# MKimiSH/video-filler

Hardware: AMD Instinct MI355X
Metric: netG+netD fwd+bwd images/sec, 128x128 center-mask (higher is better)
Workload: dtype f32

## Files before the change

video-filler_amd/csrc/vf_pgemm.hip:

```cpp
#include <algorithm>
#include <cstdlib>

#include "vf_device.h"

template <int NPL>
__global__ __launch_bounds__(256) void k_planes_split(const float* __restrict__ x, __bf16* __restrict__ planes, int64_t n4,
                                                      int64_t pstride) {
  for (int64_t i = blockIdx.x * (int64_t)blockDim.x + threadIdx.x; i < n4; i += (int64_t)gridDim.x * blockDim.x) {
    if constexpr (NPL == 1) {
      *(u32x2*)(planes + 4 * i) = vf_round4(((const f32x4*)x)[i]);
    } else {
      u32x2 o[3];
      vf_split3(((const f32x4*)x)[i], o);
#pragma unroll
      for (int q = 0; q < 3; ++q) *(u32x2*)(planes + q * pstride + 4 * i) = o[q];
    }
  }
}
__global__ __launch_bounds__(256) void k_weight_planes(const float* __restrict__ w, __bf16* __restrict__ nat, __bf16* __restrict__ tr,
                                                       int d0, int d1, int64_t pstride, int npl) {
  __shared__ float tile[32][33];
  const int t0 = blockIdx.x * 32, tap = blockIdx.y, u0 = blockIdx.z * 32;
  const int tx = threadIdx.x & 31, ty = threadIdx.x >> 5;
  for (int j = ty; j < 32; j += 8) {
// ... 511 lines not shown
    for (int g = 0; g < CH / 16; ++g) {
      const int cs = g & 1;
      if (g + 1 < CH / 16) read_frag(g + 1, cs ^ 1);
      __builtin_amdgcn_sched_barrier(0);
      if constexpr (NPL == 3) {
        acc[0][0] = __builtin_amdgcn_mfma_f32_32x32x16_bf16(a[cs][1], b[cs][1], acc[0][0], 0, 0, 0);
        acc[0][0] = __builtin_amdgcn_mfma_f32_32x32x16_bf16(a[cs][0], b[cs][2], acc[0][0], 0, 0, 0);
        acc[0][0] = __builtin_amdgcn_mfma_f32_32x32x16_bf16(a[cs][2], b[cs][0], acc[0][0], 0, 0, 0);
        acc[0][0] = __builtin_amdgcn_mfma_f32_32x32x16_bf16(a[cs][0], b[cs][1], acc[0][0], 0, 0, 0);
        acc[0][0] = __builtin_amdgcn_mfma_f32_32x32x16_bf16(a[cs][1], b[cs][0], acc[0][0], 0, 0, 0);
      }
      acc[0][0] = __builtin_amdgcn_mfma_f32_32x32x16_bf16(a[cs][0], b[cs][0], acc[0][0], 0, 0, 0);
      __builtin_amdgcn_sched_barrier(0);
    }
  };

  float pre_d[16], pre_x[16];
  const bool fin_tile = p.ksplit == 1;
  const bool want_d = fin_tile && p.dmask != nullptr, want_x = fin_tile && p.st.mode == 2;
#pragma unroll
  for (int r = 0; r < 16; ++r) {
    pre_d[r] = 1.f;
    pre_x[r] = 0.f;
  }
  if (want_d || want_x) {
    const int n = n0 + wn + lr;
    const int bw = 2 * (n >> 6) + (n & 1), bb = (n >> 1) & 31, wpp = p.N >> 5;
#pragma unroll
    for (int r = 0; r < 16; ++r) {
      const int m = m0 + wm + (r & 3) + 8 * (r >> 2) + 4 * lh;
      const int mx = m & (Mw - 1), my = (m >> p.lgMw) & (Mh - 1), b = m >> (p.lgMw + p.lgMh);
      const int64_t pix = ((int64_t)b * p.outH + (my * p.osy + ooy0)) * p.outW + (mx * p.osx + oox0);
      if (want_d) pre_d[r] = p.dbits ? (float)((p.dbits[pix * wpp + bw] >> bb) & 1u) : p.dmask[pix * p.N + n];
      if (want_x) pre_x[r] = p.st.x[pix * p.N + n];
    }
  }

  dma_step(ch0, VfIntC<0>{}, 0, ch0 < ch1);
  static_assert(NTAPS % 2 == 0, "the two LDS stages alternate with the tap parity");
  for (int ch = ch0; ch < ch1; ++ch) {
    const bool more = ch + 1 < ch1;
    asm volatile("" : "+s"(rowA), "+s"(colA), "+s"(w0), "+s"(rowW), "+s"(colW));
    vf_static_for<NTAPS>([&](auto T) {
      constexpr int t = decltype(T)::value;
      constexpr int buf = NBUF == 2 ? (t & 1) : 0, nbuf = NBUF == 2 ? (buf ^ 1) : 0;
      auto next_stage = [&]() {
        if (!(p.dbg & 1)) {
          if constexpr (t + 1 < NTAPS)
            dma_step(ch, VfIntC<t + 1>{}, nbuf, true);
          else
            dma_step(ch + 1, VfIntC<0>{}, nbuf, more);
        }
      };
      asm volatile("s_waitcnt vmcnt(0)\n\ts_barrier" ::: "memory");
      __builtin_amdgcn_sched_barrier(0);
      if constexpr (NBUF == 2) next_stage();
      __builtin_amdgcn_sched_barrier(0);
      if (!(p.dbg & 4)) compute_step(buf);
      if constexpr (NBUF == 1) {
        asm volatile("s_barrier" ::: "memory");
        next_stage();
      }
    });
  }
  asm volatile("s_waitcnt vmcnt(0)\n\ts_barrier" ::: "memory");
  pg_epilogue<1, 1, WAVES_M, BN, true>(p, acc, (float*)smem, m0, n0, wm, wn, lane, tid, wave / WAVES_N, bx, ks, ooy0, oox0, ph, pw, true,
                                       pre_d, pre_x);
}

template <int CPB>
__global__ __launch_bounds__(512) void k_pconv_patch_tr(const PGemm p) {
  constexpr int PR = CPB == 4 ? 10 : 9, PW = 18, NSLOT = PR * PW, NG = (NSLOT + 7) / 8;
  constexpr int AGW = (NG + 7) / 8;
  constexpr int PATCH_PL = NG * 8 * 128, PATCH_BYTES = 3 * PATCH_PL;
  constexpr int W_PL = 64 * 128, WBUF = 3 * W_PL;
  constexpr int NS = 4 * CPB;
  __shared__ __attribute__((aligned(1024))) unsigned char smem[PATCH_BYTES + 2 * WBUF + 2 * 4 * 64 * 4];
  float* red = (float*)(smem + PATCH_BYTES + 2 * WBUF);

  const int tid = threadIdx.x, lane = tid & 63;
  const int wave = __builtin_amdgcn_readfirstlane(tid >> 6);
  const int wm = (wave >> 1) * 32, wn = (wave & 1) * 32;
  const int lr = lane & 31, lh = lane >> 5;
  int lid = vf_xcd_remap(blockIdx.x, gridDim.x);
  const int n0 = 64 * (lid % p.gn);
  lid /= p.gn;
  int ph_blk = 0;
  if constexpr (CPB == 2) {
    ph_blk = lid & 1;
    lid >>= 1;
  }
  const int tiles_x = p.Wi >> 4, tiles_y = p.Hi >> 3;
  const int tx = lid % tiles_x, ty = (lid / tiles_x) % tiles_y, b = lid / (tiles_x * tiles_y);
  const int ry0 = 8 * ty, rx0 = 16 * tx;
  const int bx = lid;
  auto patch_sw = [](int px) { return (px >> 1) & 7; };

  unsigned a_byte[AGW], a_lds[AGW];
#pragma unroll
  for (int i = 0; i < AGW; ++i) {
    const int grp = wave + 8 * i;
    const int sl = 8 * grp + (lane >> 3);
    const int py = sl / PW, px = sl - py * PW;
    const int il = ry0 - 1 + (CPB == 2 ? ph_blk : 0) + py, jl = rx0 - 1 + px;
    const bool ok = grp < NG && sl < NSLOT && (unsigned)il < (unsigned)p.Hi && (unsigned)jl < (unsigned)p.Wi;
    const int oct = (lane & 7) ^ patch_sw(px);
    a_byte[i] = ok ? 2u * (unsigned)(((b * p.Hi + il) * p.Wi + jl) * p.C + 8 * oct) : VF_OOB;
    a_lds[i] = (unsigned)(grp * 8 * 128);
  }
  const int wrow = 8 * wave + (lane >> 3);
  const unsigned w_byte = 2u * (unsigned)((n0 + wrow) * 16 * p.C + 8 * ((lane & 7) ^ ((wrow >> 1) & 7)));
  const unsigned w_lds = (unsigned)(wave * 8 * 128);
  const __amdgpu_buffer_rsrc_t rsA = vf_rsrc(p.A, p.a_bytes), rsW = vf_rsrc(p.W, p.w_bytes);
  const unsigned lds0 = (unsigned)(uintptr_t)(__attribute__((address_space(3))) void*)smem;
  unsigned szero;
  asm volatile("s_mov_b32 %0, 0" : "=s"(szero));

  auto dma_patch = [&](int ch) {
    const unsigned cb = 128u * (unsigned)ch;
#pragma unroll
    for (int i = 0; i < AGW; ++i) {
      if (wave + 8 * i < NG) {
#pragma unroll
        for (int q = 0; q < 3; ++q)
          pg_dma16(lds0 + (unsigned)(q * PATCH_PL) + a_lds[i], a_byte[i] == VF_OOB ? VF_OOB : a_byte[i] + cb, rsA, szero + q * p.a_ps);
      }
    }
  };
  auto dma_w = [&](int ch, auto STEP, int buf) {
    constexpr int s_ = decltype(STEP)::value, cls = s_ >> 2, th = (s_ >> 1) & 1, tw = s_ & 1;
    const int ph = CPB == 4 ? (cls >> 1) : ph_blk, pw = CPB == 4 ? (cls & 1) : cls;
    const int kh = 3 - ph - 2 * th, kw = 3 - pw - 2 * tw;
    const unsigned tW = 2u * (unsigned)((kh * 4 + kw) * p.C) + 128u * (unsigned)ch;
#pragma unroll
    for (int q = 0; q < 3; ++q)
      pg_dma16(lds0 + (unsigned)(PATCH_BYTES + buf * WBUF + q * W_PL) + w_lds, w_byte, rsW, q * p.w_ps + tW);
  };

  f32x16 acc[CPB];
#pragma unroll
  for (int c = 0; c < CPB; ++c)
#pragma unroll
    for (int r = 0; r < 16; ++r) acc[c][r] = 0.f;

  const int arow = wm + lr;
  const int apy = arow >> 4, apx = arow & 15;
  int slot00 = apy * PW + apx;
  const int brow = wn + lr;
  unsigned b_off0 = (unsigned)(brow * 128);
  const unsigned b_sw = (unsigned)((brow >> 1) & 7);
  auto compute_step = [&](auto STEP, int buf) {
    constexpr int s_ = decltype(STEP)::value, cls = s_ >> 2, th = (s_ >> 1) & 1, tw = s_ & 1;
    const int ph = CPB == 4 ? (cls >> 1) : 0, pw = CPB == 4 ? (cls & 1) : cls;
    const int slot = slot00 + (ph + th) * PW + pw + tw;
    const unsigned a_off0 = (unsigned)(slot * 128), a_sw = (unsigned)patch_sw(apx + pw + tw);
    const unsigned char* wb = smem + PATCH_BYTES + buf * WBUF;
    bf16x8 a[2][3], bb[2][3];
    auto read_frag = [&](int g, int set) {
      const unsigned o = (unsigned)(2 * g + lh);
#pragma unroll
      for (int q = 0; q < 3; ++q) {
        a[set][q] = *(const bf16x8*)(smem + q * PATCH_PL + a_off0 + ((o ^ a_sw) << 4));
        bb[set][q] = *(const bf16x8*)(wb + q * W_PL + b_off0 + ((o ^ b_sw) << 4));
      }
    };
    read_frag(0, 0);
#pragma unroll
    for (int g = 0; g < 4; ++g) {
      const int cs = g & 1;
      if (g + 1 < 4) read_frag(g + 1, cs ^ 1);
      __builtin_amdgcn_sched_barrier(0);
      acc[cls] = __builtin_amdgcn_mfma_f32_32x32x16_bf16(a[cs][1], bb[cs][1], acc[cls], 0, 0, 0);
      acc[cls] = __builtin_amdgcn_mfma_f32_32x32x16_bf16(a[cs][0], bb[cs][2], acc[cls], 0, 0, 0);
      acc[cls] = __builtin_amdgcn_mfma_f32_32x32x16_bf16(a[cs][2], bb[cs][0], acc[cls], 0, 0, 0);
      acc[cls] = __builtin_amdgcn_mfma_f32_32x32x16_bf16(a[cs][0], bb[cs][1], acc[cls], 0, 0, 0);
      acc[cls] = __builtin_amdgcn_mfma_f32_32x32x16_bf16(a[cs][1], bb[cs][0], acc[cls], 0, 0, 0);
      acc[cls] = __builtin_amdgcn_mfma_f32_32x32x16_bf16(a[cs][0], bb[cs][0], acc[cls], 0, 0, 0);
      __builtin_amdgcn_sched_barrier(0);
    }
  };

  const int n = wn + lr;
  const int N = p.N;
  const int stm = p.st.mode;
  const bool want_d = p.dmask != nullptr, want_x = stm == 2;
  const float bv = p.bias ? p.bias[n0 + n] : 0.f;
  const float sv = stm ? p.st.vec[(stm == 2 ? (bx / p.st.tiles_per_group) * N : 0) + n0 + n] : 0.f;
  const float neg = p.act == VF_ACT_LRELU ? p.slope : (p.act == VF_ACT_RELU ? 0.f : 1.f);
  const float dneg = p.dact == VF_ACT_LRELU ? p.dslope : (p.dact == VF_ACT_RELU ? 0.f : 1.f);
  const unsigned ybytes = (unsigned)(p.out_elems * 4);
  const __amdgpu_buffer_rsrc_t rsY = vf_rsrc(p.Y, ybytes), rsD = vf_rsrc(p.dbits ? (const void*)p.dbits : (const void*)p.dmask, p.dbits ? ybytes / 32 : ybytes),
                               rsX = vf_rsrc(p.st.x, ybytes);
  unsigned pix0 = (unsigned)(((b * p.outH + 2 * (ry0 + 2 * (wave >> 1))) * p.outW) + 2 * (rx0 + 4 * lh));
  const unsigned ostride = (unsigned)(2 * p.outW);
  float pre_d[16], pre_x[16];
  auto pixel = [&](int r, int ph, int pw) -> unsigned {
    return pix0 + (unsigned)(ph * p.outW + pw) + (unsigned)(r >> 3) * ostride + (unsigned)(2 * ((r & 3) + 8 * ((r >> 2) & 1)));
  };
  auto elem = [&](int r, int ph, int pw) -> unsigned { return pixel(r, ph, pw) * (unsigned)N + (unsigned)(n0 + n); };
  auto prefetch_epi = [&](int ph, int pw) {
#pragma unroll
    for (int r = 0; r < 16; ++r) {
      const unsigned px_ = pixel(r, ph, pw), e = px_ * (unsigned)N + (unsigned)(n0 + n);
      pre_d[r] = 1.f;
      pre_x[r] = 0.f;
      if (want_d) {
        if (p.dbits)
          pre_d[r] = (float)((__builtin_amdgcn_raw_buffer_load_b32(rsD, 4u * (px_ * (unsigned)(N >> 5) + (unsigned)(2 * (n0 >> 6) + (n & 1))), 0, 0) >> ((n >> 1) & 31)) & 1u);
        else pre_d[r] = __builtin_bit_cast(float, __builtin_amdgcn_raw_buffer_load_b32(rsD, 4u * e, 0, 0));
      }
      if (want_x) pre_x[r] = __builtin_bit_cast(float, __builtin_amdgcn_raw_buffer_load_b32(rsX, 4u * e, 0, 0));
    }
  };
  auto epilogue = [&](auto CLS, int ph, int pw) {
    constexpr int cls = decltype(CLS)::value;
    float st1[1] = {0.f}, st2[1] = {0.f};
#pragma unroll
    for (int r = 0; r < 16; ++r) {
      float v = acc[cls][r] + bv;
      v = v * (v > 0.f ? 1.f : neg);
      if (want_d) v = v * (pre_d[r] > 0.f ? 1.f : dneg);
      if (stm == 1) {
        const float d = v - sv;
        st1[0] += d;
        st2[0] += d * d;
      } else if (stm == 2) {
        st1[0] += v;
        st2[0] += v * (pre_x[r] - sv);
      }
      acc[cls][r] = v;
    }
    if (stm) vf_bn_tile_partials<1, 4, 64>(p.st, st1, st2, red, wave >> 1, wn, lane, tid, n0, N, bx, (ph << 1) | pw);
  };
  auto store_class = [&](auto CLS, int ph, int pw) {
    constexpr int cls = decltype(CLS)::value;
#pragma unroll
    for (int r = 0; r < 16; ++r) {
      const float v = acc[cls][r];
      if (!(p.dbg & 8)) __builtin_amdgcn_raw_buffer_store_b32(__builtin_bit_cast(unsigned, v), rsY, 4u * elem(r, ph, pw), 0, 0);
    }
  };

  const int nch = p.nchunks;
  dma_patch(0);
  dma_w(0, VfIntC<0>{}, 0);
  for (int ch = 0; ch < nch; ++ch) {
    const bool last = ch + 1 == nch;
    asm volatile("" : "+v"(slot00), "+v"(b_off0), "+v"(pix0));
    vf_static_for<NS>([&](auto S) {
      constexpr int s_ = decltype(S)::value, buf = s_ & 1, cls = s_ >> 2, tap = s_ & 3;
      const int ph = CPB == 4 ? (cls >> 1) : ph_blk, pw = CPB == 4 ? (cls & 1) : cls;
      asm volatile("s_waitcnt vmcnt(0)\n\ts_barrier" ::: "memory");
      __builtin_amdgcn_sched_barrier(0);
      if (!(p.dbg & 1)) {
        if constexpr (s_ + 1 < NS) dma_w(ch, VfIntC<s_ + 1>{}, buf ^ 1);
        else if (!last) dma_w(ch + 1, VfIntC<0>{}, buf ^ 1);
      }
      if (last && tap == 0 && (want_d || want_x)) prefetch_epi(ph, pw);
      __builtin_amdgcn_sched_barrier(0);
      if (!(p.dbg & 4)) compute_step(S, buf);
      if (last && tap == 3) epilogue(VfIntC<cls>{}, ph, pw);
    });
    if (!last) {
      asm volatile("s_barrier" ::: "memory");
      dma_patch(ch + 1);
    }
  }
  vf_static_for<CPB>([&](auto C) {
    constexpr int cls = decltype(C)::value;
    store_class(C, CPB == 4 ? (cls >> 1) : ph_blk, CPB == 4 ? (cls & 1) : cls);
  });
}

template <int MODE, bool TR = false>
__global__ __launch_bounds__(512) void k_pconv_patch_g(const PGemm p) {
  static_assert(!TR || MODE != 0, "the transposed form serves whole-map tiles (8 x 16 regions of larger maps: k_pconv_patch_tr)");
  constexpr int NS = TR ? 4 : 16;
  constexpr int PW = 17;
  constexpr int NSLOT = MODE == 0 ? 9 * PW : 130;
  constexpr int NG = (NSLOT + 7) / 8, AGW = (NG + 7) / 8;
  constexpr int PL = NG * 8 * 128;
  constexpr int W_PL = 64 * 128, WBUF = 3 * W_PL;
  constexpr int OFF_LO = 4 * PL, OFF_W = 5 * PL;
  __shared__ __attribute__((aligned(1024))) unsigned char smem[5 * PL + 2 * WBUF];
  float* red = (float*)(smem + OFF_W);

  const int tid = threadIdx.x, lane = tid & 63;
  const int wave = __builtin_amdgcn_readfirstlane(tid >> 6);
  const int wm = (wave >> 1) * 32, wn = (wave & 1) * 32;
  const int lr = lane & 31, lh = lane >> 5;
  const int ntiles = p.gm * p.gn * p.gz;
  int lid = vf_xcd_remap(blockIdx.x, ntiles);
  int ph = 0, pw = 0;
  if constexpr (TR) {
    ph = (lid >> 1) & 1;
    pw = lid & 1;
    lid >>= 2;
  }
  const int bx = lid % p.gm, byz = lid / p.gm;
  const int n0 = (byz % p.gn) * 64;
  const int ks = byz / p.gn;
  const int cps = p.nchunks / p.ksplit;
  const int ch0 = ks * cps;
  const int Wo = 1 << p.lgMw, Ho = 1 << p.lgMh;

  int b_img = 0, oy0 = 0, ox0 = 0;
  if constexpr (MODE == 0) {
    const int tiles_x = Wo >> 4, tiles_y = Ho >> 3;
    const int tx = bx % tiles_x, ty = (bx / tiles_x) % tiles_y;
    b_img = bx / (tiles_x * tiles_y);
    oy0 = 8 * ty;
    ox0 = 16 * tx;
  }
  constexpr int HW = MODE == 1 ? 64 : 16, LW = MODE == 1 ? 3 : 2;

  unsigned a_byte[AGW], a_ok[AGW], a_lds[AGW];
#pragma unroll
  for (int i = 0; i < AGW; ++i) {
    const int grp = wave + 8 * i;
    const int sl = 8 * grp + (lane >> 3);
    a_lds[i] = (unsigned)(grp * 8 * 128);
    if constexpr (MODE == 0) {
      const int r = sl / PW, c = sl - r * PW;
      const int y00 = 2 * (oy0 + r) - 1, x00 = 2 * (ox0 + c) - 1;
      const int oct = (lane & 7) ^ (c & 7);
      a_byte[i] = 2u * (unsigned)(((b_img * p.Hi + y00) * p.Wi + x00) * p.C + 8 * oct);
      unsigned ok = 0;
#pragma unroll
      for (int cls = 0; cls < 4; ++cls)
        if ((unsigned)(y00 + (cls >> 1)) < (unsigned)p.Hi && (unsigned)(x00 + (cls & 1)) < (unsigned)p.Wi) ok |= 1u << cls;
      a_ok[i] = (grp < NG && sl < NSLOT) ? ok : 0u;
    } else {
      const int g = sl >> (2 * LW), ii = (sl >> LW) & (Wo - 1), jj = sl & (Wo - 1);
      const int oct = (lane & 7) ^ ((sl >> 1) & 7);
      const int img = bx * (128 / HW) + g;
      if constexpr (TR) a_byte[i] = 2u * (unsigned)(((img * p.Hi + ii) * p.Wi + jj) * p.C + 8 * oct);
      else a_byte[i] = 2u * (unsigned)(((img * p.Hi + 2 * ii + 1) * p.Wi + 2 * jj + 1) * p.C + 8 * oct);
      a_ok[i] = (grp < NG && sl < 128) ? 15u : 0u;
    }
  }
  const int wrow = 8 * wave + (lane >> 3);
  const unsigned w_byte = 2u * (unsigned)((n0 + wrow) * 16 * p.C + 8 * ((lane & 7) ^ ((wrow >> 1) & 7)));
  const unsigned w_lds = (unsigned)(wave * 8 * 128);
  const __amdgpu_buffer_rsrc_t rsA = vf_rsrc(p.A, p.a_bytes), rsW = vf_rsrc(p.W, p.w_bytes);
  const unsigned lds0 = (unsigned)(uintptr_t)(__attribute__((address_space(3))) void*)smem;
  unsigned szero;
  asm volatile("s_mov_b32 %0, 0" : "=s"(szero));
  int rowA = 2 * p.Wi * p.C, colA = 2 * p.C;

  auto dma_patch_plane = [&](int ch, int cls, int pb, auto Q, bool live) {
    constexpr int q = decltype(Q)::value;
    const int cth = cls >> 1, ctw = cls & 1;
    const unsigned cb = 128u * (unsigned)ch + (TR ? 0u : (unsigned)(MODE == 0 ? cth * rowA + ctw * colA : -(cth * rowA + ctw * colA)));
    const unsigned dst = lds0 + (unsigned)(q == 2 ? OFF_LO : (2 * pb + q) * PL);
// ... 373 lines not shown
          acc[nt] = __builtin_amdgcn_mfma_f32_32x32x16_bf16(a1[0], b1[0][nt], acc[nt], 0, 0, 0);
        }
      }
    } else {
    bf16x8 a[2][NPL], b[2][NPL][2];
    auto read_frag = [&](int g, int set) {
#pragma unroll
      for (int q = 0; q < NPL; ++q) {
        a[set][q] = pg_tr_frag(base + q * PL_SZ, wm, 16 * g, lane);
#pragma unroll
        for (int nt = 0; nt < 2; ++nt) b[set][q][nt] = pg_tr_frag(base + q * PL_SZ + TILE, wn + 32 * nt, 16 * g, lane);
      }
    };
    read_frag(0, 0);
#pragma unroll
    for (int g = 0; g < BK / 16; ++g) {
      const int cs = g & 1;
      if (g + 1 < BK / 16) read_frag(g + 1, cs ^ 1);
      __builtin_amdgcn_sched_barrier(0);
#pragma unroll
      for (int nt = 0; nt < 2; ++nt) {
        if constexpr (NPL == 3) {
          acc[nt] = __builtin_amdgcn_mfma_f32_32x32x16_bf16(a[cs][1], b[cs][1][nt], acc[nt], 0, 0, 0);
          acc[nt] = __builtin_amdgcn_mfma_f32_32x32x16_bf16(a[cs][0], b[cs][2][nt], acc[nt], 0, 0, 0);
          acc[nt] = __builtin_amdgcn_mfma_f32_32x32x16_bf16(a[cs][2], b[cs][0][nt], acc[nt], 0, 0, 0);
          acc[nt] = __builtin_amdgcn_mfma_f32_32x32x16_bf16(a[cs][0], b[cs][1][nt], acc[nt], 0, 0, 0);
          acc[nt] = __builtin_amdgcn_mfma_f32_32x32x16_bf16(a[cs][1], b[cs][0][nt], acc[nt], 0, 0, 0);
        }
        acc[nt] = __builtin_amdgcn_mfma_f32_32x32x16_bf16(a[cs][0], b[cs][0][nt], acc[nt], 0, 0, 0);
      }
      __builtin_amdgcn_sched_barrier(0);
    }
    }
  };

  if (fed32) {
    for (int kt = kt0; kt < kt1; ++kt) {
      stage_fp32(kt);
      __syncthreads();
      compute_stage();
      __syncthreads();
    }
  } else {
    for (int kt = kt0; kt < kt1; ++kt) {
      dma_stage(kt);
      asm volatile("s_waitcnt vmcnt(0)\n\ts_barrier" ::: "memory");
      __builtin_amdgcn_sched_barrier(0);
      compute_stage();
      asm volatile("s_barrier" ::: "memory");
    }
  }

  const int lr = lane & 31, lh = lane >> 5;
  const int64_t total = (int64_t)p.Nu * Ncols;
  float* out = p.out + (p.ksplit > 1 ? (int64_t)ks * total : 0);
  const bool acc_old = p.ksplit == 1 && p.beta != 0.f;
#pragma unroll
  for (int r = 0; r < 16; ++r) {
    const int n = n0 + wm + (r & 3) + 8 * (r >> 2) + 4 * lh;
    if (n >= p.Nu) continue;
#pragma unroll
    for (int nt = 0; nt < 2; ++nt) {
      const int64_t idx = (int64_t)n * Ncols + j0 + wn + nt * 32 + lr;
      float v = acc[nt][r];
      if (acc_old) v += p.beta * out[idx];
      out[idx] = v;
    }
  }
}

int vf_internal_pwgrad_group(vf_ctx* ctx, const VfPWGradGroup& G, int blocks, const char* name, double flops) {
  if (ctx->mfma_bf16 == 1)
    VF_LAUNCH_TIMED(ctx, "pwgrad_group_128x128x32_bf16", flops, 0.0, (k_pwgrad_group<1, 2>), dim3((unsigned)blocks), dim3(512), G);
  else
    VF_LAUNCH_TIMED(ctx, name, flops, 0.0, (k_pwgrad_group<3, 1>), dim3((unsigned)blocks), dim3(512), G);
  VF_LAUNCH_CHECK();
  return 0;
}

static int g_gather_patch = 1;
static int g_scatter_patch = 1;
VF_API int vf_pconv_set_routing(int gather_patch, int scatter_patch) {
  if (gather_patch >= 0) g_gather_patch = gather_patch != 0;
  if (scatter_patch >= 0) g_scatter_patch = scatter_patch != 0;
  return 0;
}

typedef void (*PgKernel)(PGemm);

template <int BM, int NTAPS>
static PgKernel pg_dma_kernel(bool one_plane, bool one_stage) {
  if (one_plane) return k_pconv_dma<BM, 64, NTAPS, 2, 1>;
  return one_stage ? k_pconv_dma<BM, 64, NTAPS, 1> : k_pconv_dma<BM, 64, NTAPS, 2>;
}

template <int BM, int WM, int NTAPS>
static PgKernel pg_reg_kernel(int ch) {
  return ch == 64 ? k_pconv<BM, 64, WM, 32, NTAPS, 64> : k_pconv<BM, 64, WM, 32, NTAPS, 32>;
}

static int launch_pconv(vf_ctx* ctx, PGemm& g, int ntaps, VfConvExtras* ex) {
  const int zpar = g.parity ? 4 : 1;
  const int ch = g.C % 64 == 0 ? 64 : 32;
  g.nchunks = g.C / ch;
  constexpr int bn = 64;
  const bool dma_shape = ch == 64 && g.N % bn == 0;
  const int bm = dma_shape ? (g.M % 128 == 0 ? 128 : 64) : (vf_cdiv(g.M, 128) * vf_cdiv(g.N, bn) * zpar >= 1024 ? 128 : 64);
  const bool use_dma = dma_shape && g.M % bm == 0;
  const int gm = (int)vf_cdiv(g.M, bm), gn = (int)vf_cdiv(g.N, bn);
  const int64_t blocks = (int64_t)gm * gn * zpar;
  constexpr int SPLIT_BLOCKS = 340;
  int ksplit = 1;
  if (blocks < SPLIT_BLOCKS * 3 / 4 && g.nchunks >= 2) {
    ksplit = (int)std::min<int64_t>(g.nchunks, vf_cdiv(SPLIT_BLOCKS, blocks));
    const size_t slab_bytes = (size_t)g.out_elems * sizeof(float);
    while (ksplit > 1 && (size_t)ksplit * slab_bytes > vf_ws_avail(ctx)) --ksplit;
    while (ksplit > 1 && g.nchunks % ksplit != 0) --ksplit;
  }
  g.ksplit = ksplit;
  g.slab = ksplit > 1 ? (float*)vf_ws_ptr(ctx) : nullptr;
  g.gm = gm; g.gn = gn; g.gz = zpar * ksplit;
  const unsigned nt = (unsigned)(blocks * ksplit);
  const bool slab_st = vf_plan_bn_stats(ex, g, bm, gm, zpar);
  const bool one_plane = ctx->mfma_bf16 == 1;
  VF_REQUIRE(!one_plane || use_dma, "vf_pconv: in the bf16-operand mode the planes path serves whole 64-channel / 64-row tiles only "
             "(vf_pconv_supported_in_mode)");

  const char* taps = ntaps == 16 ? "t16" : "t4";
  const double fl = 2.0 * (double)g.M * g.N * (double)ntaps * g.C * zpar;
  const double dby = (double)g.a_bytes + (double)g.w_bytes + 4.0 * (double)g.out_elems * ksplit +
                     (g.dmask ? (g.dbits ? 0.125 : 4.0) * (double)g.out_elems : 0.0) + (g.st.mode == 2 ? 4.0 * (double)g.out_elems : 0.0);
  char name[64];
  PgKernel kern;
  dim3 grid(nt), block(bm == 128 ? 512 : 256);
  double by = dby;
  const int Ho = 1 << g.lgMh, Wo = 1 << g.lgMw;
  const int gmode = (Wo % 16 == 0 && Ho % 8 == 0) ? 0 : (Ho == 8 && Wo == 8) ? 1 : (Ho == 4 && Wo == 4) ? 2 : -1;
  if (use_dma && one_plane) {
    snprintf(name, sizeof(name), "pconv_dma_%dx%dx64_%s_bf16", bm, bn, taps);
    kern = bm == 128 ? (ntaps == 16 ? pg_dma_kernel<128, 16>(true, false) : pg_dma_kernel<128, 4>(true, false))
                     : (ntaps == 16 ? pg_dma_kernel<64, 16>(true, false) : pg_dma_kernel<64, 4>(true, false));
  } else if (use_dma && g_scatter_patch && ntaps == 4 && g.parity && ksplit == 1 && bm == 128 && g.Wi % 16 == 0 && g.Hi % 8 == 0 &&
             (g.act == VF_ACT_NONE || g.act == VF_ACT_LRELU || g.act == VF_ACT_RELU) &&
             g.out_elems * 4 < ((int64_t)1 << 31)) {
    const unsigned tiles = (unsigned)(g.M / 128), slices = (unsigned)(g.N / 64);
    const int cpb = tiles * slices >= 512 ? 4 : 2;
    snprintf(name, sizeof(name), "pconv_patch_128x64_t4_c%d", cpb);
    grid = dim3(tiles * slices * (cpb == 2 ? 2u : 1u));
    kern = cpb == 4 ? k_pconv_patch_tr<4> : k_pconv_patch_tr<2>;
  } else if (use_dma && g_gather_patch && ntaps == 16 && !g.parity && bm == 128 && g.sy == 2 && g.sx == 2 && gmode >= 0) {
    snprintf(name, sizeof(name), "pconv_patchg_128x64_t16_m%d", gmode);
    kern = gmode == 0 ? k_pconv_patch_g<0> : gmode == 1 ? k_pconv_patch_g<1> : k_pconv_patch_g<2>;
  } else if (use_dma && g_scatter_patch && ntaps == 4 && g.parity && bm == 128 && nt < 512 &&
             ((g.Hi == 8 && g.Wi == 8) || (g.Hi == 4 && g.Wi == 4))) {
    const int mode = g.Hi == 8 ? 1 : 2;
    snprintf(name, sizeof(name), "pconv_patchg_128x64_t4_m%d", mode);
    kern = mode == 1 ? k_pconv_patch_g<1, true> : k_pconv_patch_g<2, true>;
  } else if (use_dma) {
    const bool one_stage = bm == 128 && nt >= 512;
    snprintf(name, sizeof(name), "pconv_dma_%dx%dx64_%s%s", bm, bn, taps, one_stage ? "_1stage" : "");
    kern = bm == 128 ? (ntaps == 16 ? pg_dma_kernel<128, 16>(false, one_stage) : pg_dma_kernel<128, 4>(false, one_stage))
                     : (ntaps == 16 ? pg_dma_kernel<64, 16>(false, one_stage) : pg_dma_kernel<64, 4>(false, one_stage));
  } else {
    snprintf(name, sizeof(name), "pconv_%dx%dx%d_%s", bm, bn, ch, taps);
    kern = bm == 128 ? (ntaps == 16 ? pg_reg_kernel<128, 64, 16>(ch) : pg_reg_kernel<128, 64, 4>(ch))
                     : (ntaps == 16 ? pg_reg_kernel<64, 32, 16>(ch) : pg_reg_kernel<64, 32, 4>(ch));
    block = dim3(256);
    by = 0.0;
  }

  VF_LAUNCH_TIMED(ctx, name, fl, by, kern, grid, block, g);
  VF_LAUNCH_CHECK();
  if (ksplit > 1) {
    VfProf prof(ctx, slab_st ? "slab_reduce_pconv_bnstats" : "slab_reduce_pconv", 0.0, 4.0 * (double)g.out_elems * (ksplit + 1));
    return vf_internal_slab_reduce(ctx, g.slab, g.Y, g.bias, g.out_elems, g.N, ksplit, g.act, g.slope, g.dmask, g.dact, g.dslope,
                                   slab_st ? &g.st : nullptr, slab_st ? ex->bn.groups : 1);
  }
  return 0;
}

static int pg_fill_common(vf_ctx* ctx, PGemm& g, const void* a, const void* w, const float* bias, float* y, const VfConvShape& s) {
  memset(&g, 0, sizeof(g));
  g.A = a; g.W = w; g.bias = bias; g.Y = y;
  g.Hi = s.H; g.Wi = s.W; g.C = s.Cin; g.N = s.Cout;
  const int64_t a_elems = (int64_t)s.B * s.H * s.W * s.Cin, w_elems = (int64_t)s.Cout * 16 * s.Cin;
  const int npl = ctx->mfma_bf16 == 1 ? 1 : 3;
  VF_REQUIRE(ctx->mfma_bf16 == 3 || ctx->mfma_bf16 == 1, "vf_pconv: the planes path serves product modes 3 (exact split) and 1 (bf16 operands)");
  VF_REQUIRE(a_elems * 2 * npl < ((int64_t)1 << 31) && w_elems * 2 * npl < ((int64_t)1 << 31), "planes exceed the 2 GiB buffer-descriptor range");
  g.a_ps = (unsigned)(a_elems * 2);
  g.w_ps = (unsigned)(w_elems * 2);
  g.a_bytes = npl * g.a_ps;
  g.w_bytes = npl * g.w_ps;
  return 0;
}

static int pconv_like_fwd(vf_ctx* ctx, const void* ap, const void* wp, const float* bias, float* Y, const VfConvShape& s, int act,
                          float slope, VfConvExtras* ex) {
  const int Ho = s.H / 2, Wo = s.W / 2;
  PGemm g;
  if (int rc = pg_fill_common(ctx, g, ap, wp, bias, Y, s)) return rc;
  g.lgMh = vf_ilog2(Ho); g.lgMw = vf_ilog2(Wo);
  g.M = s.B * Ho * Wo;
  g.sy = 2; g.oy0 = -1; g.sx = 2; g.ox0 = -1;
  g.lgTW = 2;
  g.kh0 = 0; g.khs = 1; g.kw0 = 0; g.kws = 1;
  g.outH = Ho; g.outW = Wo; g.osy = 1; g.osx = 1;
  g.out_elems = (int64_t)g.M * s.Cout;
  g.act = act; g.slope = slope;
  return launch_pconv(ctx, g, 16, ex);
}
static int pconv_like_tr(vf_ctx* ctx, const void* ap, const void* wp, const float* bias, float* Y, const VfConvShape& s, int act,
                         float slope, const float* dmask, int dact, float dslope, VfConvExtras* ex) {
  PGemm g;
  if (int rc = pg_fill_common(ctx, g, ap, wp, bias, Y, s)) return rc;
  g.lgMh = vf_ilog2(s.H); g.lgMw = vf_ilog2(s.W);
  g.M = s.B * s.H * s.W;
  g.sy = 1; g.oy0 = -1; g.sx = 1; g.ox0 = -1;
  g.lgTW = 1;
  g.khs = -2; g.kws = -2;
  g.parity = 1;
  g.outH = 2 * s.H; g.outW = 2 * s.W; g.osy = 2; g.osx = 2;
  g.out_elems = (int64_t)s.B * g.outH * g.outW * s.Cout;
  g.act = act; g.slope = slope;
  g.dmask = dmask; g.dact = dact; g.dslope = dslope;
  g.dbits = (dmask && s.Cout % 64 == 0) ? ex->dmask_bits : nullptr;
  return launch_pconv(ctx, g, 4, ex);
}

VF_API int vf_planes_split(vf_ctx* ctx, const float* x, void* planes, int64_t n) {
  VF_REQUIRE(n % 4 == 0 && vf_aligned16(x) && ((uintptr_t)planes & 7) == 0, "vf_planes_split: n %% 4 == 0 and aligned buffers");
  const int64_t n4 = n / 4;
// ... 65 lines not shown
```

Baseline: 24000.

## Process two tiles per block in patch transposed-conv and overlap stores with compute

The scatter-patch transposed-conv kernel becomes persistent over up to two adjacent work units, launching half the blocks when there are at least 512 units. The next unit's patch and weight DMA is issued before the previous unit's final store. Stores of each finished parity class are interleaved into the next class's MFMA steps instead of a trailing store loop. The mask-bit extraction moves into the epilogue. The routing knob gains forcing modes that pick the CPB variant and disable k-split, at the cost of more complex waitcnt bookkeeping.

```diff
diff --git a/video-filler_amd/csrc/vf_pgemm.hip b/video-filler_amd/csrc/vf_pgemm.hip
--- a/video-filler_amd/csrc/vf_pgemm.hip
+++ b/video-filler_amd/csrc/vf_pgemm.hip
@@ -617,34 +617,46 @@
   const int wave = __builtin_amdgcn_readfirstlane(tid >> 6);
   const int wm = (wave >> 1) * 32, wn = (wave & 1) * 32;
   const int lr = lane & 31, lh = lane >> 5;
-  int lid = vf_xcd_remap(blockIdx.x, gridDim.x);
-  const int n0 = 64 * (lid % p.gn);
-  lid /= p.gn;
-  int ph_blk = 0;
-  if constexpr (CPB == 2) {
-    ph_blk = lid & 1;
-    lid >>= 1;
-  }
-  const int tiles_x = p.Wi >> 4, tiles_y = p.Hi >> 3;
-  const int tx = lid % tiles_x, ty = (lid / tiles_x) % tiles_y, b = lid / (tiles_x * tiles_y);
-  const int ry0 = 8 * ty, rx0 = 16 * tx;
-  const int bx = lid;
+  constexpr bool ADJACENT = true;
+  const int nunits = p.gm * p.gn * (CPB == 2 ? 2 : 1);
+  const int upb = nunits > (int)gridDim.x ? 2 : 1;
+  int unit = (ADJACENT ? upb : 1) * vf_xcd_remap(blockIdx.x, gridDim.x);
+  const int unit_step = ADJACENT ? 1 : (int)gridDim.x;
+  int units_left = upb;
+  int n0, ph_blk, b, ry0, rx0, bx;
+  auto decode = [&](int lid) {
+    n0 = 64 * (lid % p.gn);
+    lid /= p.gn;
+    ph_blk = 0;
+    if constexpr (CPB == 2) {
+      ph_blk = lid & 1;
+      lid >>= 1;
+    }
+    const int tiles_x = p.Wi >> 4, tiles_y = p.Hi >> 3;
+    const int tx = lid % tiles_x, ty = (lid / tiles_x) % tiles_y;
+    b = lid / (tiles_x * tiles_y);
+    ry0 = 8 * ty;
+    rx0 = 16 * tx;
+    bx = lid;
+  };
   auto patch_sw = [](int px) { return (px >> 1) & 7; };
 
-  unsigned a_byte[AGW], a_lds[AGW];
-#pragma unroll
-  for (int i = 0; i < AGW; ++i) {
-    const int grp = wave + 8 * i;
-    const int sl = 8 * grp + (lane >> 3);
-    const int py = sl / PW, px = sl - py * PW;
-    const int il = ry0 - 1 + (CPB == 2 ? ph_blk : 0) + py, jl = rx0 - 1 + px;
-    const bool ok = grp < NG && sl < NSLOT && (unsigned)il < (unsigned)p.Hi && (unsigned)jl < (unsigned)p.Wi;
-    const int oct = (lane & 7) ^ patch_sw(px);
-    a_byte[i] = ok ? 2u * (unsigned)(((b * p.Hi + il) * p.Wi + jl) * p.C + 8 * oct) : VF_OOB;
-    a_lds[i] = (unsigned)(grp * 8 * 128);
-  }
+  unsigned a_byte[AGW], a_lds[AGW], w_byte;
   const int wrow = 8 * wave + (lane >> 3);
-  const unsigned w_byte = 2u * (unsigned)((n0 + wrow) * 16 * p.C + 8 * ((lane & 7) ^ ((wrow >> 1) & 7)));
+  auto aim = [&]() {
+#pragma unroll
+    for (int i = 0; i < AGW; ++i) {
+      const int grp = wave + 8 * i;
+      const int sl = 8 * grp + (lane >> 3);
+      const int py = sl / PW, px = sl - py * PW;
+      const int il = ry0 - 1 + (CPB == 2 ? ph_blk : 0) + py, jl = rx0 - 1 + px;
+      const bool ok = grp < NG && sl < NSLOT && (unsigned)il < (unsigned)p.Hi && (unsigned)jl < (unsigned)p.Wi;
+      const int oct = (lane & 7) ^ patch_sw(px);
+      a_byte[i] = ok ? 2u * (unsigned)(((b * p.Hi + il) * p.Wi + jl) * p.C + 8 * oct) : VF_OOB;
+      a_lds[i] = (unsigned)(grp * 8 * 128);
+    }
+    w_byte = 2u * (unsigned)((n0 + wrow) * 16 * p.C + 8 * ((lane & 7) ^ ((wrow >> 1) & 7)));
+  };
   const unsigned w_lds = (unsigned)(wave * 8 * 128);
   const __amdgpu_buffer_rsrc_t rsA = vf_rsrc(p.A, p.a_bytes), rsW = vf_rsrc(p.W, p.w_bytes);
   const unsigned lds0 = (unsigned)(uintptr_t)(__attribute__((address_space(3))) void*)smem;
@@ -673,10 +685,6 @@
   };
 
   f32x16 acc[CPB];
-#pragma unroll
-  for (int c = 0; c < CPB; ++c)
-#pragma unroll
-    for (int r = 0; r < 16; ++r) acc[c][r] = 0.f;
 
   const int arow = wm + lr;
   const int apy = arow >> 4, apx = arow & 15;
@@ -719,92 +727,137 @@
   const int N = p.N;
   const int stm = p.st.mode;
   const bool want_d = p.dmask != nullptr, want_x = stm == 2;
-  const float bv = p.bias ? p.bias[n0 + n] : 0.f;
-  const float sv = stm ? p.st.vec[(stm == 2 ? (bx / p.st.tiles_per_group) * N : 0) + n0 + n] : 0.f;
+  float bv, sv;
   const float neg = p.act == VF_ACT_LRELU ? p.slope : (p.act == VF_ACT_RELU ? 0.f : 1.f);
   const float dneg = p.dact == VF_ACT_LRELU ? p.dslope : (p.dact == VF_ACT_RELU ? 0.f : 1.f);
   const unsigned ybytes = (unsigned)(p.out_elems * 4);
   const __amdgpu_buffer_rsrc_t rsY = vf_rsrc(p.Y, ybytes), rsD = vf_rsrc(p.dbits ? (const void*)p.dbits : (const void*)p.dmask, p.dbits ? ybytes / 32 : ybytes),
                                rsX = vf_rsrc(p.st.x, ybytes);
-  unsigned pix0 = (unsigned)(((b * p.outH + 2 * (ry0 + 2 * (wave >> 1))) * p.outW) + 2 * (rx0 + 4 * lh));
+  unsigned pix0;
   const unsigned ostride = (unsigned)(2 * p.outW);
-  float pre_d[16], pre_x[16];
-  auto pixel = [&](int r, int ph, int pw) -> unsigned {
-    return pix0 + (unsigned)(ph * p.outW + pw) + (unsigned)(r >> 3) * ostride + (unsigned)(2 * ((r & 3) + 8 * ((r >> 2) & 1)));
-  };
-  auto elem = [&](int r, int ph, int pw) -> unsigned { return pixel(r, ph, pw) * (unsigned)N + (unsigned)(n0 + n); };
-  auto prefetch_epi = [&](int ph, int pw) {
+  const int nch = p.nchunks;
+  decode(unit);
+  aim();
+  dma_patch(0);
+  dma_w(0, VfIntC<0>{}, 0);
+  for (bool carried = false;; carried = true) {
+    float pre_d[16], pre_x[16];
 #pragma unroll
     for (int r = 0; r < 16; ++r) {
-      const unsigned px_ = pixel(r, ph, pw), e = px_ * (unsigned)N + (unsigned)(n0 + n);
       pre_d[r] = 1.f;
       pre_x[r] = 0.f;
+    }
+    auto pixel = [&](int r, int ph, int pw) -> unsigned {
+      return pix0 + (unsigned)(ph * p.outW + pw) + (unsigned)(r >> 3) * ostride + (unsigned)(2 * ((r & 3) + 8 * ((r >> 2) & 1)));
+    };
+    auto prefetch_epi = [&](int ph, int pw) {
       if (want_d) {
-        if (p.dbits)
-          pre_d[r] = (float)((__builtin_amdgcn_raw_buffer_load_b32(rsD, 4u * (px_ * (unsigned)(N >> 5) + (unsigned)(2 * (n0 >> 6) + (n & 1))), 0, 0) >> ((n >> 1) & 31)) & 1u);
-        else pre_d[r] = __builtin_bit_cast(float, __builtin_amdgcn_raw_buffer_load_b32(rsD, 4u * e, 0, 0));
-      }
-      if (want_x) pre_x[r] = __builtin_bit_cast(float, __builtin_amdgcn_raw_buffer_load_b32(rsX, 4u * e, 0, 0));
-    }
-  };
-  auto epilogue = [&](auto CLS, int ph, int pw) {
-    constexpr int cls = decltype(CLS)::value;
-    float st1[1] = {0.f}, st2[1] = {0.f};
-#pragma unroll
-    for (int r = 0; r < 16; ++r) {
-      float v = acc[cls][r] + bv;
-      v = v * (v > 0.f ? 1.f : neg);
-      if (want_d) v = v * (pre_d[r] > 0.f ? 1.f : dneg);
-      if (stm == 1) {
-        const float d = v - sv;
-        st1[0] += d;
-        st2[0] += d * d;
-      } else if (stm == 2) {
-        st1[0] += v;
-        st2[0] += v * (pre_x[r] - sv);
-      }
-      acc[cls][r] = v;
-    }
-    if (stm) vf_bn_tile_partials<1, 4, 64>(p.st, st1, st2, red, wave >> 1, wn, lane, tid, n0, N, bx, (ph << 1) | pw);
-  };
-  auto store_class = [&](auto CLS, int ph, int pw) {
-    constexpr int cls = decltype(CLS)::value;
-#pragma unroll
-    for (int r = 0; r < 16; ++r) {
-      const float v = acc[cls][r];
-      if (!(p.dbg & 8)) __builtin_amdgcn_raw_buffer_store_b32(__builtin_bit_cast(unsigned, v), rsY, 4u * elem(r, ph, pw), 0, 0);
-    }
-  };
-
-  const int nch = p.nchunks;
-  dma_patch(0);
-  dma_w(0, VfIntC<0>{}, 0);
-  for (int ch = 0; ch < nch; ++ch) {
-    const bool last = ch + 1 == nch;
-    asm volatile("" : "+v"(slot00), "+v"(b_off0), "+v"(pix0));
-    vf_static_for<NS>([&](auto S) {
-      constexpr int s_ = decltype(S)::value, buf = s_ & 1, cls = s_ >> 2, tap = s_ & 3;
-      const int ph = CPB == 4 ? (cls >> 1) : ph_blk, pw = CPB == 4 ? (cls & 1) : cls;
-      asm volatile("s_waitcnt vmcnt(0)\n\ts_barrier" ::: "memory");
-      __builtin_amdgcn_sched_barrier(0);
-      if (!(p.dbg & 1)) {
-        if constexpr (s_ + 1 < NS) dma_w(ch, VfIntC<s_ + 1>{}, buf ^ 1);
-        else if (!last) dma_w(ch + 1, VfIntC<0>{}, buf ^ 1);
-      }
-      if (last && tap == 0 && (want_d || want_x)) prefetch_epi(ph, pw);
-      __builtin_amdgcn_sched_barrier(0);
-      if (!(p.dbg & 4)) compute_step(S, buf);
-      if (last && tap == 3) epilogue(VfIntC<cls>{}, ph, pw);
-    });
-    if (!last) {
+        if (p.dbits) {
+#pragma unroll
+          for (int r = 0; r < 16; ++r)
+            pre_d[r] = __builtin_bit_cast(float, __builtin_amdgcn_raw_buffer_load_b32(rsD, 4u * (pixel(r, ph, pw) * (unsigned)(N >> 5) + (unsigned)(2 * (n0 >> 6) + (n & 1))), 0, 0));
+        } else {
+#pragma unroll
+          for (int r = 0; r < 16; ++r)
+            pre_d[r] = __builtin_bit_cast(float, __builtin_amdgcn_raw_buffer_load_b32(rsD, 4u * (pixel(r, ph, pw) * (unsigned)N + (unsigned)(n0 + n)), 0, 0));
+        }
+      }
+      if (want_x) {
+#pragma unroll
+        for (int r = 0; r < 16; ++r)
+          pre_x[r] = __builtin_bit_cast(float, __builtin_amdgcn_raw_buffer_load_b32(rsX, 4u * (pixel(r, ph, pw) * (unsigned)N + (unsigned)(n0 + n)), 0, 0));
+      }
+    };
+    auto epilogue = [&](auto CLS, int ph, int pw) {
+      constexpr int cls = decltype(CLS)::value;
+      float st1[1] = {0.f}, st2[1] = {0.f};
+#pragma unroll
+      for (int r = 0; r < 16; ++r) {
+        float v = acc[cls][r] + bv;
+        v = v * (v > 0.f ? 1.f : neg);
+        if (want_d) v = v * ((p.dbits ? ((__builtin_bit_cast(unsigned, pre_d[r]) >> ((n >> 1) & 31)) & 1u) != 0u : pre_d[r] > 0.f) ? 1.f : dneg);
+        if (stm == 1) {
+          const float d = v - sv;
+          st1[0] += d;
+          st2[0] += d * d;
+        } else if (stm == 2) {
+          st1[0] += v;
+          st2[0] += v * (pre_x[r] - sv);
+        }
+        acc[cls][r] = v;
+      }
+      if (stm) vf_bn_tile_partials<1, 4, 64>(p.st, st1, st2, red, wave >> 1, wn, lane, tid, n0, N, bx, (ph << 1) | pw);
+    };
+    constexpr bool SPREAD = false;
+    constexpr int ST = SPREAD ? 4 : 16;
+    auto store_rows = [&](auto CLS, auto R0, auto CNT, unsigned pixb, unsigned col, int ph, int pw) {
+      constexpr int cls = decltype(CLS)::value, r0 = decltype(R0)::value, cnt = decltype(CNT)::value;
+#pragma unroll
+      for (int r = r0; r < r0 + cnt; ++r) {
+        const float v = acc[cls][r];
+        const unsigned px_ = pixb + (unsigned)(ph * p.outW + pw) + (unsigned)(r >> 3) * ostride + (unsigned)(2 * ((r & 3) + 8 * ((r >> 2) & 1)));
+        __builtin_amdgcn_raw_buffer_store_b32(__builtin_bit_cast(unsigned, v), rsY, 4u * (px_ * (unsigned)N + col), 0, 0);
+      }
+    };
+    auto head = [&](auto CNT) { asm volatile("s_waitcnt vmcnt(%0)\n\ts_barrier" ::"n"(decltype(CNT)::value) : "memory"); };
+
+    bv = p.bias ? p.bias[n0 + n] : 0.f;
+    sv = stm ? p.st.vec[(stm == 2 ? (bx / p.st.tiles_per_group) * N : 0) + n0 + n] : 0.f;
+    pix0 = (unsigned)(((b * p.outH + 2 * (ry0 + 2 * (wave >> 1))) * p.outW) + 2 * (rx0 + 4 * lh));
+#pragma unroll
+    for (int c = 0; c < CPB; ++c)
+#pragma unroll
+      for (int r = 0; r < 16; ++r) acc[c][r] = 0.f;
+    for (int ch = 0; ch < nch; ++ch) {
+      const bool last = ch + 1 == nch;
+      asm volatile("" : "+v"(slot00), "+v"(b_off0), "+v"(pix0));
+      vf_static_for<NS>([&](auto S) {
+        constexpr int s_ = decltype(S)::value, buf = s_ & 1, cls = s_ >> 2, tap = s_ & 3;
+        constexpr int st_here = (cls >= 1 && (SPREAD || tap == 0)) ? ST : 0;
+        constexpr int st_prev = (s_ >= 1 && ((s_ - 1) >> 2) >= 1 && (SPREAD || ((s_ - 1) & 3) == 0)) ? ST : 0;
+        const int ph = CPB == 4 ? (cls >> 1) : ph_blk, pw = CPB == 4 ? (cls & 1) : cls;
+        if constexpr (s_ == 0) {
+          if (carried && ch == 0) head(VfIntC<16>{});
+          else head(VfIntC<0>{});
+        } else if constexpr (st_prev > 0) {
+          if (last) head(VfIntC<st_prev>{});
+          else head(VfIntC<0>{});
+        } else {
+          head(VfIntC<0>{});
+        }
+        __builtin_amdgcn_sched_barrier(0);
+        if (!(p.dbg & 1)) {
+          if constexpr (s_ + 1 < NS) dma_w(ch, VfIntC<s_ + 1>{}, buf ^ 1);
+          else if (!last) dma_w(ch + 1, VfIntC<0>{}, buf ^ 1);
+        }
+        if (last && tap == 0 && (want_d || want_x)) prefetch_epi(ph, pw);
+        if constexpr (st_here > 0) {
+          if (last)
+            store_rows(VfIntC<(cls >= 1 ? cls - 1 : 0)>{}, VfIntC<(SPREAD ? 4 * tap : 0)>{}, VfIntC<ST>{}, pix0, (unsigned)(n0 + n),
+                       CPB == 4 ? ((cls - 1) >> 1) : ph_blk, CPB == 4 ? ((cls - 1) & 1) : cls - 1);
+        }
+        __builtin_amdgcn_sched_barrier(0);
+        if (!(p.dbg & 4)) compute_step(S, buf);
+        if (last && tap == 3) epilogue(VfIntC<cls>{}, ph, pw);
+      });
+      if (!last) {
+        asm volatile("s_barrier" ::: "memory");
+        dma_patch(ch + 1);
+      }
+    }
+    const unsigned s_pix = pix0, s_col = (unsigned)(n0 + n);
+    const int s_ph = CPB == 4 ? 1 : ph_blk;
+    const bool more = --units_left > 0 && (unit += unit_step) < nunits;
+    if (more) {
+      decode(unit);
+      aim();
       asm volatile("s_barrier" ::: "memory");
-      dma_patch(ch + 1);
-    }
-  }
-  vf_static_for<CPB>([&](auto C) {
-    constexpr int cls = decltype(C)::value;
-    store_class(C, CPB == 4 ? (cls >> 1) : ph_blk, CPB == 4 ? (cls & 1) : cls);
-  });
+      dma_patch(0);
+      dma_w(0, VfIntC<0>{}, 0);
+    }
+    store_rows(VfIntC<CPB - 1>{}, VfIntC<0>{}, VfIntC<16>{}, s_pix, s_col, s_ph, 1);
+    if (!more) break;
+  }
 }
 
 template <int MODE, bool TR = false>
@@ -1344,7 +1397,7 @@
 static int g_scatter_patch = 1;
 VF_API int vf_pconv_set_routing(int gather_patch, int scatter_patch) {
   if (gather_patch >= 0) g_gather_patch = gather_patch != 0;
-  if (scatter_patch >= 0) g_scatter_patch = scatter_patch != 0;
+  if (scatter_patch >= 0) g_scatter_patch = scatter_patch <= 7 ? scatter_patch : 1;
   return 0;
 }
 
@@ -1373,7 +1426,10 @@
   const int64_t blocks = (int64_t)gm * gn * zpar;
   constexpr int SPLIT_BLOCKS = 340;
   int ksplit = 1;
-  if (blocks < SPLIT_BLOCKS * 3 / 4 && g.nchunks >= 2) {
+  const bool patch_tr_shape = use_dma && ntaps == 4 && g.parity && bm == 128 && g.Wi % 16 == 0 && g.Hi % 8 == 0 && ctx->mfma_bf16 != 1 &&
+                              (g.act == VF_ACT_NONE || g.act == VF_ACT_LRELU || g.act == VF_ACT_RELU) && g.out_elems * 4 < ((int64_t)1 << 31);
+  const bool patch_tr_forced = g_scatter_patch >= 2 && patch_tr_shape;
+  if (blocks < SPLIT_BLOCKS * 3 / 4 && g.nchunks >= 2 && !patch_tr_forced) {
     ksplit = (int)std::min<int64_t>(g.nchunks, vf_cdiv(SPLIT_BLOCKS, blocks));
     const size_t slab_bytes = (size_t)g.out_elems * sizeof(float);
     while (ksplit > 1 && (size_t)ksplit * slab_bytes > vf_ws_avail(ctx)) --ksplit;
@@ -1402,13 +1458,14 @@
     snprintf(name, sizeof(name), "pconv_dma_%dx%dx64_%s_bf16", bm, bn, taps);
     kern = bm == 128 ? (ntaps == 16 ? pg_dma_kernel<128, 16>(true, false) : pg_dma_kernel<128, 4>(true, false))
                      : (ntaps == 16 ? pg_dma_kernel<64, 16>(true, false) : pg_dma_kernel<64, 4>(true, false));
-  } else if (use_dma && g_scatter_patch && ntaps == 4 && g.parity && ksplit == 1 && bm == 128 && g.Wi % 16 == 0 && g.Hi % 8 == 0 &&
-             (g.act == VF_ACT_NONE || g.act == VF_ACT_LRELU || g.act == VF_ACT_RELU) &&
-             g.out_elems * 4 < ((int64_t)1 << 31)) {
+  } else if (g_scatter_patch && patch_tr_shape && ksplit == 1) {
     const unsigned tiles = (unsigned)(g.M / 128), slices = (unsigned)(g.N / 64);
-    const int cpb = tiles * slices >= 512 ? 4 : 2;
+    const int force = g_scatter_patch;
+    const int cpb = force >= 2 && force <= 5 ? (force >= 4 ? 4 : 2) : (tiles * slices >= 512 ? 4 : 2);
+    const unsigned units = tiles * slices * (cpb == 2 ? 2u : 1u);
+    const bool two = force >= 2 ? (force & 1) && units >= 2 : units >= 512;
     snprintf(name, sizeof(name), "pconv_patch_128x64_t4_c%d", cpb);
-    grid = dim3(tiles * slices * (cpb == 2 ? 2u : 1u));
+    grid = dim3(two ? (units + 1) / 2 : units);
     kern = cpb == 4 ? k_pconv_patch_tr<4> : k_pconv_patch_tr<2>;
   } else if (use_dma && g_gather_patch && ntaps == 16 && !g.parity && bm == 128 && g.sy == 2 && g.sx == 2 && gmode >= 0) {
     snprintf(name, sizeof(name), "pconv_patchg_128x64_t16_m%d", gmode);
```

Result: no change. 24140, median of 5 (+0.6%).
